# j-moralejo-pinas/dist_classicrl

Measured on AMD Instinct MI355X. Metric: env-steps/sec at 128 agents, 1e6x16 Q-table; 1/2/4/8 GPU + HBM GB/s %peak, higher is better.
Workload: dtype f32

## Files before the change

### dist_classicrl_amd/csrc/qe_rollout_lane.h

```cpp
#pragma once
#include "qe_kernels.h"

namespace qe {

constexpr int LANE_MAX_AGENTS = 512;

template <typename T, int NV>
struct RowV {
    T v[4 * NV];
};

template <int NV>
struct LaneMask {
    using type = uint32_t;
};
template <>
struct LaneMask<16> {
    using type = uint64_t;
};

__device__ __forceinline__ int popc_mask(uint32_t x) { return __popc(x); }
__device__ __forceinline__ int popc_mask(uint64_t x) { return __popcll(x); }

template <int NV>
__device__ __forceinline__ void load_row_lane(RowV<float, NV>& r, const float* q, int64_t row) {
    const float4* p = reinterpret_cast<const float4*>(q + row * (4 * NV));
#pragma unroll
    for (int k = 0; k < NV; ++k) {
        const float4 f = p[k];
        r.v[4 * k] = f.x; r.v[4 * k + 1] = f.y; r.v[4 * k + 2] = f.z; r.v[4 * k + 3] = f.w;
    }
}
template <int NV>
__device__ __forceinline__ void load_row_lane(RowV<double, NV>& r, const double* q, int64_t row) {
    const double2* p = reinterpret_cast<const double2*>(q + row * (4 * NV));
#pragma unroll
    for (int k = 0; k < NV; ++k) {
        const double2 a = p[2 * k], b = p[2 * k + 1];
        r.v[4 * k] = a.x; r.v[4 * k + 1] = a.y; r.v[4 * k + 2] = b.x; r.v[4 * k + 3] = b.y;
    }
}

__device__ __forceinline__ float lane_fmax(float a, float b) { return __builtin_fmaxf(a, b); }
__device__ __forceinline__ double lane_fmax(double a, double b) { return __builtin_fmax(a, b); }

template <bool MASKED, typename T, int NV, typename M>
__device__ __forceinline__ RowV<T, NV> masked_row(const RowV<T, NV>& row, M valid) {
    if constexpr (!MASKED) {
        return row;
    } else {
        RowV<T, NV> r;
#pragma unroll
        for (int j = 0; j < 4 * NV; ++j) r.v[j] = ((valid >> j) & 1) ? row.v[j] : neg_inf<T>();
        return r;
    }
}

template <typename T, int NV>
__device__ __forceinline__ T row_max_lane(const RowV<T, NV>& rowm) {
    T m = neg_inf<T>();
#pragma unroll
    for (int j = 0; j < 4 * NV; ++j) m = lane_fmax(m, rowm.v[j]);
    return m;
}

template <int NV>
__device__ __forceinline__ bool row_nan_lane(const RowV<float, NV>& rowm) {
    typedef float f2 __attribute__((ext_vector_type(2)));
    f2 acc0 = {0.0f, 0.0f}, acc1 = {0.0f, 0.0f};
#pragma unroll
    for (int j = 0; j < 4 * NV; j += 4) {
        const f2 x = {rowm.v[j], rowm.v[j + 1]}, y = {rowm.v[j + 2], rowm.v[j + 3]};
        acc0 = __builtin_elementwise_fma(x, x, acc0);
        acc1 = __builtin_elementwise_fma(y, y, acc1);
    }
    const f2 acc = acc0 + acc1;
    const float s = acc.x + acc.y;
    return s != s;
}
template <int NV>
__device__ __forceinline__ bool row_nan_lane(const RowV<double, NV>& rowm) {
    double acc = 0.0;
#pragma unroll
    for (int j = 0; j < 4 * NV; ++j) acc += rowm.v[j] * rowm.v[j];
    return acc != acc;
}
template <typename T, int NV>
__device__ __forceinline__ T row_max_np_lane(const RowV<T, NV>& rowm) {
    const T m = row_max_lane(rowm);
    return row_nan_lane<NV>(rowm) ? quiet_nan<T>() : m;
}

template <typename T, int NV, int LO, int CNT>
__device__ __forceinline__ T row_pick_tree(const RowV<T, NV>& row, int idx) {
    constexpr int W = 4 * NV;
    if constexpr (CNT == 1) {
        T x = row.v[LO < W ? LO : W - 1];
        asm volatile("" : "+v"(x));
        return x;
    } else {
        const T lo = row_pick_tree<T, NV, LO, CNT / 2>(row, idx);
        const T hi = row_pick_tree<T, NV, LO + CNT / 2, CNT / 2>(row, idx);
        T r = (idx & (CNT / 2)) ? hi : lo;
        asm volatile("" : "+v"(r));
        return r;
    }
}
template <typename T, int NV>
__device__ __forceinline__ T row_pick_lane(const RowV<T, NV>& row, int idx) {
    constexpr int W = 4 * NV;
    constexpr int P = W <= 4 ? 4 : (W <= 8 ? 8 : (W <= 16 ? 16 : (W <= 32 ? 32 : 64)));
    return row_pick_tree<T, NV, 0, P>(row, idx);
}

template <int NV, typename M>
__device__ __forceinline__ int kth_set_bit(M f, int k) {
    constexpr int W = 4 * NV;
    constexpr int P = W <= 4 ? 4 : (W <= 8 ? 8 : (W <= 16 ? 16 : (W <= 32 ? 32 : 64)));
    constexpr int LOG = P == 4 ? 2 : (P == 8 ? 3 : (P == 16 ? 4 : (P == 32 ? 5 : 6)));
    int pos = 0;
#pragma unroll
    for (int lv = 0; lv < LOG; ++lv) {
        const int width = P >> (lv + 1);
        const M low = f & (((M)1 << width) - 1);
        const int c = popc_mask(low);
        const bool hi = k >= c;
        k -= hi ? c : 0;
        f = hi ? (f >> width) : low;
        pos += hi ? width : 0;
    }
    return pos;
}

template <typename T, int NV, typename M, bool PICK = true>
__device__ __forceinline__ int select_lane(const RowV<T, NV>& rowm, M valid, bool explore, uint32_t x1,
                                           uint32_t x2, T* picked, bool nan_max) {
    T m = row_max_lane(rowm);
    if (nan_max) m = quiet_nan<T>();
    M ties = 0;
#pragma unroll
    for (int j = 0; j < 4 * NV; ++j) ties |= (M)(rowm.v[j] == m ? 1u : 0u) << j;
    const M f = explore ? valid : (ties & valid);
    const int total = popc_mask(f);
    int act = -1;
    if (total > 0) act = kth_set_bit<NV>(f, (int)mulhi32(explore ? x1 : x2, (uint32_t)total));
    if constexpr (PICK) *picked = row_pick_lane(rowm, act < 0 ? 0 : act);
    return act;
}

template <class Env, int NV, bool MASKED>
__device__ __forceinline__ typename LaneMask<NV>::type valid_mask_lane(const EnvCtx& ev, int64_t i, int32_t obs) {
    using M = typename LaneMask<NV>::type;
    if constexpr (!MASKED) {
        return ev.A >= 8 * (int)sizeof(M) ? ~(M)0 : (((M)1 << ev.A) - 1);
    } else {
        M m = 0;
#pragma unroll
        for (int sub = 0; sub < NV; ++sub) m |= (M)Env::valid4(ev, i, obs, sub) << (4 * sub);
        return m;
    }
}

template <int CAP>
struct LaneCfg {
    static constexpr int WT = CAP <= 128 ? 4096 : 2048;
    static constexpr int BT = 2048;
};

template <int CAP, bool HELP>
struct LaneLds {
    SlowLdsT<CAP, PERSIST_CACHE_BYTES> slow;
    int wt[4][LaneCfg<CAP>::WT + 1];
    int bt_key[LaneCfg<CAP>::BT];
    unsigned bt_cnt[LaneCfg<CAP>::BT];
    int bt_min[LaneCfg<CAP>::BT];
    uint32_t draws[2][3][HELP ? CAP : 1];
    unsigned long long ep_key[EP_STAGE];
    float ep_ret[EP_STAGE];
    unsigned char pending[CAP];
    alignas(16) unsigned char cold[448];
    unsigned def_bits[CAP / 32];
    unsigned busy[5];
    unsigned ep_n;
    unsigned n_def;
    unsigned complex_;
    int seq_min[2];
};

struct alignas(16) SchedSlot {
    double lr;
    unsigned long long thr;
};
template <int CAP>
struct LaneLdsSlim : LaneLds<CAP, true> {
    SchedSlot sched[2];
    uint2 acct[2][CAP];
};

__device__ __forceinline__ float opaque_copy(float v) {
    float r;
    asm volatile("v_mov_b32 %0, %1" : "=v"(r) : "v"(v));
    return r;
}
__device__ __forceinline__ double opaque_copy(double v) {
    double r;
    asm volatile("v_mov_b64 %0, %1" : "=v"(r) : "v"(v));
    return r;
}

#ifdef QE_EXPERIMENT
#define QX(bit) ((flags >> (20 + (bit))) & 1)
#else
#define QX(bit) 0
#endif
#ifdef QE_STAMPS
#define QL_STAMP(k) do { const long long _n = wall_clock64(); stamp_sum[k] += _n - stamp_last; stamp_last = _n; } while (0)
#else
#define QL_STAMP(k) do { } while (0)
#endif

template <int PENDING_LOADS>
__device__ __forceinline__ void step_barrier() {
    if constexpr (PENDING_LOADS == 0) asm volatile("s_waitcnt vmcnt(0) lgkmcnt(0)\n\ts_barrier" ::: "memory");
    else asm volatile("s_waitcnt vmcnt(%0) lgkmcnt(0)\n\ts_barrier" ::"n"(PENDING_LOADS) : "memory");
}

template <typename T, class Env, int NV, int CAP, bool MASKED, int LEAN = 0, bool HELP = false, bool FULL = false,
          bool SEQ = false>
__global__ __launch_bounds__(HELP ? 4 * CAP : CAP) void k_rollout_lane(InlineSched ,
                                                                       Ctx<T> c, EnvCtx ev, long long steps, int flags) {
    using M = typename LaneMask<NV>::type;
    constexpr int NLOAD = NV * (int)(sizeof(T) / 4);
    constexpr int WT = LaneCfg<CAP>::WT, BT = LaneCfg<CAP>::BT;
    constexpr bool SLIM = HELP && SEQ && FULL && LEAN != 0;
    __shared__ std::conditional_t<SLIM, LaneLdsSlim<CAP>, LaneLds<CAP, HELP>> lds;
    const unsigned long long clk0 = wall_clock64();
    const unsigned long long cyc0 = __builtin_amdgcn_s_memtime();
    if (c.thr == nullptr) {
        const QE_AS4 unsigned char* ka = (const QE_AS4 unsigned char*)__builtin_amdgcn_kernarg_segment_ptr();
        c.thr = (const QE_AS4 unsigned long long*)ka;
        c.lr = (const QE_AS4 double*)(ka + sizeof(unsigned long long) * INLINE_SCHED_STEPS);
    }
    if constexpr (LEAN != 0) { c.mode = 0; c.trace = nullptr; c.rp.s = nullptr; }
    if constexpr (LEAN == 1) c.dlog = nullptr;
#ifdef QE_STAMPS
    long long stamp_sum[8] = {0, 0, 0, 0, 0, 0, 0, 0};
    long long stamp_last = wall_clock64();
    if (threadIdx.x == 0) for (int k = 8; k < 24; ++k) c.vinc[k] = 0.0;
#endif
    const int tid = threadIdx.x;
    const int n_main = HELP ? (int)((c.N + 63) & ~63ll) : (int)blockDim.x;
    const int wave_tid = __builtin_amdgcn_readfirstlane(tid);
    const bool helper = HELP && wave_tid >= n_main && wave_tid < 2 * n_main;
    const bool worker = HELP && wave_tid >= 2 * n_main;
    const int i = helper ? tid - n_main : (worker ? 0 : tid);
    const bool active = FULL ? !(helper || worker) : (!(helper || worker) && i < c.N);
    const int ii = i < c.N ? i : 0;
    Pending<T> p;
    p.n = c.n[ii];
    p.aux = c.aux[ii];
    p.s = 0; p.a = 0; p.pred = 0; p.r = 0.0f; p.term = false;
    float acc = c.acc[ii];
    unsigned long long deferred_total = 0, ep_base = 0;
    unsigned complex_steps = 0;
    int w_next = WT, w_cur = WT, w_prev = WT;
    const int flush_every = 32;
    int flush_in = flush_every;
    for (int k = tid; k < 4 * (WT + 1); k += (int)blockDim.x) (&lds.wt[0][0])[k] = -1;
    for (int k = tid; k < BT; k += (int)blockDim.x) { lds.bt_key[k] = -1; lds.bt_cnt[k] = 0u; lds.bt_min[k] = 0x7FFFFFFF; }
    for (int k = tid; k < CAP; k += (int)blockDim.x) lds.pending[k] = 0;
    if (tid < CAP / 32) lds.def_bits[tid] = 0u;
    static_assert(sizeof(Ctx<T>) <= sizeof(lds.cold), "context stash too small");
    if (tid == 0) {
        *reinterpret_cast<Ctx<T>*>(lds.cold) = c;
        lds.ep_n = 0u; lds.n_def = 0u; lds.complex_ = 0u;
        lds.seq_min[0] = 0x7FFFFFFF; lds.seq_min[1] = 0x7FFFFFFF;
        for (int k = 0; k < 5; ++k) lds.busy[k] = 0u;
        c.ctrl->error = 0u;
        c.ctrl->inv_count = 0u;
    }
    __syncthreads();
    if ((QX(6) && worker) || (QX(7) && helper)) return;

    const bool nan_sel = c.nan_select != 0;
    auto advance = [&](const RowV<T, NV>& row, M valid, long long t1, const U4& x, unsigned long long thr_t1, bool row_nan) {
        const bool explore = (unsigned long long)x.x < thr_t1;
        T picked = p.pred;
        int act = select_lane<T, NV, M, !SLIM>(masked_row<MASKED>(row, valid), valid, explore, x.y, x.z, &picked, nan_sel && row_nan);
        if (act < 0) {
            c.ctrl->error = ERR_EMPTY_CHOICE;
            act = 0;
        }
        const int32_t n = p.n;
        const Transition tr = Env::step(ev, i, n, p.aux, act, c.step0 + (unsigned long long)t1);
        if (c.trace) c.trace[t1 * c.N + i] = act;
        replay_put(c, t1, i, n, act, tr.reward, tr.next_obs, tr.terminated);
        p.s = n; p.a = act; p.pred = picked; p.r = tr.reward; p.term = tr.terminated; p.n = tr.next_obs;
    };
    auto philox_of = [&](long long t1) {
        const unsigned long long step1 = c.step0 + (unsigned long long)t1;
        return philox4x32_10(c.agent_offset + (uint32_t)ii, (uint32_t)step1, (uint32_t)(step1 >> 32), STREAM_POLICY,
                             c.seed_lo, c.seed_hi);
    };
    auto draws = [&](long long t1) {
        if constexpr (HELP) {
            const int slot = (int)(t1 & 1);
            return U4{lds.draws[slot][0][ii], lds.draws[slot][1][ii], lds.draws[slot][2][ii], 0u};
        } else {
            return philox_of(t1);
        }
    };
    auto produce = [&](long long t1) {
        const U4 x = philox_of(t1);
        const int slot = (int)(t1 & 1);
        lds.draws[slot][0][ii] = x.x; lds.draws[slot][1][ii] = x.y; lds.draws[slot][2][ii] = x.z;
        if constexpr (SLIM) {
            if (tid == n_main) {
                lds.sched[slot].lr = c.lr[t1 - 1];
                lds.sched[slot].thr = c.thr[t1 < steps ? t1 : (steps > 0 ? steps - 1 : 0)];
            }
        }
    };
    auto helper_account = [&](long long tk) {
        if constexpr (SLIM) {
            const uint2 rt = lds.acct[tk & 1][ii];
            const bool term = rt.y != 0u;
            acc += __uint_as_float(rt.x);
            const bool ends = term && (flags & FLAG_ACCOUNT);
            const unsigned long long enders = __ballot(ends);
            const float ep_value = acc;
            if (term) acc = 0.0f;
            if (enders) {
                const unsigned rank = __builtin_amdgcn_mbcnt_hi((unsigned)(enders >> 32), __builtin_amdgcn_mbcnt_lo((unsigned)enders, 0u));
                unsigned ep_raw = 0;
                if (ends && rank == 0) ep_raw = atomicAdd(&lds.ep_n, (unsigned)__popcll(enders));
                const unsigned base = __builtin_amdgcn_readlane(ep_raw, __ffsll((long long)enders) - 1);
                if (ends) {
                    const unsigned ep_slot = base + rank;
                    const unsigned long long key = ((unsigned long long)tk << 32) | (unsigned long long)ii;
                    if (ep_slot < (unsigned)EP_STAGE) {
                        lds.ep_key[ep_slot] = key;
                        lds.ep_ret[ep_slot] = ep_value;
                    } else {
                        const Ctx<T>& cc = *reinterpret_cast<const Ctx<T>*>(lds.cold);
                        if ((long long)(ep_base + ep_slot) < cc.ep_cap) {
                            cc.ep_key[ep_base + ep_slot] = key;
                            cc.ep_ret[ep_base + ep_slot] = ep_value;
                        }
                    }
                }
            }
        }
    };
    auto bookkeeping = [&](long long k, bool check_stale) {
        int* const tab_w = lds.wt[(k + 1) & 3];
        const int* const tab_r = lds.wt[k & 3];
        const int* const tab_st = lds.wt[(k + 3) & 3];
        const int32_t rowid = p.n;
        const int h = (int)(mix32((uint32_t)rowid) & (WT - 1));
        const bool need_r = rowid != p.s;
        int o_w = atomicCAS(&tab_w[h], -1, rowid);
        int k_r = need_r ? tab_r[h] : -1;
        int k_st = check_stale ? tab_st[h] : -1;
        int h_w = h, h_r = h, h_st = h;
        bool odd_w = o_w != -1 && o_w != rowid, odd_r = k_r != -1 && k_r != rowid, odd_st = k_st != -1 && k_st != rowid;
        while (__any(odd_w || odd_r || odd_st)) {
            h_w = odd_w ? (h_w + 1) & (WT - 1) : h_w;
            h_r = (h_r + 1) & (WT - 1);
            h_st = (h_st + 1) & (WT - 1);
            const int o2 = atomicCAS(&tab_w[odd_w ? h_w : WT], odd_w ? -1 : -2, rowid);
            const int r2 = tab_r[odd_r ? h_r : WT];
            const int s2 = tab_st[odd_st ? h_st : WT];
            o_w = odd_w ? o2 : o_w; k_r = odd_r ? r2 : k_r; k_st = odd_st ? s2 : k_st;
            odd_w = o_w != -1 && o_w != rowid; odd_r = k_r != -1 && k_r != rowid; odd_st = k_st != -1 && k_st != rowid;
        }
        lds.busy[o_w == rowid ? (int)((k + 1) & 3) : 4] = 1u;
        lds.busy[k_r == rowid ? (int)(k & 3) : 4] = 1u;
        w_prev = w_cur; w_cur = w_next; w_next = h_w;
        return k_st == rowid;
    };

    RowV<T, NV> row;
    bool stale = false;
    T* pred_cell = c.q;
    T pred_pend = 0;
    {
        load_row_lane<NV>(row, c.q, p.n);
        if (active) {
            const M valid0 = valid_mask_lane<Env, NV, MASKED>(ev, i, p.n);
            advance(row, valid0, 0, philox_of(0), c.thr[0], row_nan_lane<NV>(masked_row<MASKED>(row, valid0)));
            int h = (int)(mix32((uint32_t)p.s) & (WT - 1));
            int old = atomicCAS(&lds.wt[0][h], -1, p.s);
            while (old != -1 && old != p.s) {
                h = (h + 1) & (WT - 1);
                old = atomicCAS(&lds.wt[0][h], -1, p.s);
            }
            if (old == p.s) lds.busy[0] = 1u;
            w_next = h;
        }
        if (helper) produce(1);
        __syncthreads();
        if (active) (void)bookkeeping(0, false);
        load_row_lane<NV>(row, c.q, p.n);
        if constexpr (SLIM) {
            pred_cell = c.q + ((int64_t)p.s * (4 * NV) + p.a);
            pred_pend = *pred_cell;
        }
        if constexpr (SLIM) if (active) lds.acct[0][i] = make_uint2(__float_as_uint(p.r), p.term ? 1u : 0u);
    }
    __syncthreads();
    DeltaEntry* dl = c.dlog ? c.dlog + c.dlog_base + ii : nullptr;
    const long long dl_steps = c.dlog ? (c.dlog_cap - c.dlog_base) / c.N : 0;
    int vzero = 0;
    if constexpr (!SLIM) asm volatile("v_mov_b32 %0, 0" : "=v"(vzero));
    double lr_pend = 0.0;
    unsigned long long thr_pend = 0;
    if constexpr (!SLIM) {
        lr_pend = ((const double*)(uintptr_t)c.lr)[vzero];
        thr_pend = ((const unsigned long long*)(uintptr_t)c.thr)[(steps > 1 ? 1 : 0) + vzero];
    }
    for (long long t = 0; t < steps; ++t) {
        const bool last = t + 1 == steps;
        const bool dl_ok = t < dl_steps;
        QL_STAMP(7);
        const bool busy = lds.busy[t & 3] != 0u;
        const U4 x = draws(t + 1);
        double lr_ring = 0.0;
        unsigned long long thr_ring = 0;
        if constexpr (SLIM) { lr_ring = lds.sched[(t + 1) & 1].lr; thr_ring = lds.sched[(t + 1) & 1].thr; }
        if (helper && !last && !QX(5)) produce(t + 2);
        if constexpr (SLIM) if (helper) helper_account(t);
        if (stale && !QX(8)) load_row_lane<NV>(row, c.q, p.n);
        const M valid = valid_mask_lane<Env, NV, MASKED>(ev, ii, p.n);
        QL_STAMP(0);
        int cls = 3;
        int pred_s = -1, pred_n = -1;
        int b_s = -1, b_n = -1;
        if (busy) {
            if (active) {
                auto bt_insert = [&](int32_t rowid) {
                    int h = (int)(mix32((uint32_t)rowid) & (BT - 1));
                    for (;;) {
                        const int old = atomicCAS(&lds.bt_key[h], -1, rowid);
                        if (old == -1 || old == rowid) return h;
                        h = (h + 1) & (BT - 1);
                    }
                };
                b_s = bt_insert(p.s);
                atomicAdd(&lds.bt_cnt[b_s], 1u << 16);
                atomicMin(&lds.bt_min[b_s], i);
                if (p.n != p.s) {
                    b_n = bt_insert(p.n);
                    atomicAdd(&lds.bt_cnt[b_n], 1u);
                    atomicMin(&lds.bt_min[b_n], i);
                }
            }
            barrier_lds();
            if (active) {
                const unsigned cs = lds.bt_cnt[b_s];
                const int ms = lds.bt_min[b_s];
                unsigned cn = 0u;
                int mn = 0x7FFFFFFF;
                const bool has_n = b_n >= 0;
                if (has_n) { cn = lds.bt_cnt[b_n]; mn = lds.bt_min[b_n]; }
                const unsigned w_s = cs >> 16, tot_s = w_s + (cs & 0xFFFFu);
                const unsigned w_n = cn >> 16, tot_n = w_n + (cn & 0xFFFFu);
                bool now = true, sel = true, cx = false;
                if (c.mode == 1) {
                    const bool shared = w_s >= 2u || (w_s == 1u && tot_s >= 2u) || (has_n && w_n >= 1u && tot_n >= 2u);
                    if (shared) { now = false; cx = true; }
                    sel = !(has_n ? w_n > 0u : w_s > 1u);
                } else {
                    if (tot_s > 1u && ms < i) { now = false; pred_s = ms; cx |= tot_s > 2u; }
                    if (has_n) {
                        if (w_n > 0u) {
                            sel = false;
                            if (!p.term && mn < i) { now = false; pred_n = mn; cx |= tot_n > 2u; }
                        }
                    } else if (w_s > 1u) {
                        sel = false;
                    }
                }
                cls = (now ? 1 : 0) | (sel ? 2 : 0);
                if (!now) {
                    lds.pending[i] = 1;
                    atomicAdd(&lds.n_def, 1u);
                    if (cx) lds.complex_ = 1u;
                }
            }
        }
        QL_STAMP(2);
        __builtin_amdgcn_s_waitcnt(0x0F70);
        double lr_t;
        unsigned long long thr_t1;
        if constexpr (SLIM) {
            lr_t = lr_ring;
            thr_t1 = thr_ring;
        } else {
            asm volatile("v_mov_b64 %0, %1" : "=v"(lr_t) : "v"(lr_pend));
            asm volatile("v_mov_b64 %0, %1" : "=v"(thr_t1) : "v"(thr_pend));
            lr_pend = ((const double*)(uintptr_t)c.lr)[(last ? t : t + 1) + vzero];
            thr_pend = ((const unsigned long long*)(uintptr_t)c.thr)[(t + 2 < steps ? t + 2 : steps - 1) + vzero];
        }
        if constexpr (SLIM) p.pred = opaque_copy(pred_pend);
        const float r_t = p.r;
        const bool term_t = p.term;
        bool row_nan = row_nan_lane<NV>(masked_row<MASKED>(row, valid));
        if (active && (cls & 1)) {
            T m = row_max_lane(masked_row<MASKED>(row, valid));
            if (row_nan) m = quiet_nan<T>();
            const int64_t cell = (int64_t)p.s * (4 * NV) + p.a;
            T u;
            const T q1 = Td<T>::apply(p.pred, p.r, m, p.term, make_hyper(c, lr_t), c.mode, &u);
            if (p.n == p.s) row_nan |= q1 != q1;
            if constexpr (SLIM) *pred_cell = q1;
            else if (!QX(1)) c.q[cell] = q1;
            if (dl_ok) *dl = DeltaEntry{(uint32_t)cell, (float)u};
            if (p.n == p.s) {
#pragma unroll
                for (int j = 0; j < 4 * NV; ++j) row.v[j] = j == p.a ? q1 : row.v[j];
            }
        }
        unsigned ep_raw = 0;
        unsigned long long enders = 0;
        float ep_value = 0.0f;
        if (!SLIM && active) {
            acc += r_t;
            enders = __ballot(term_t && (flags & FLAG_ACCOUNT));
            const unsigned rank = __builtin_amdgcn_mbcnt_hi((unsigned)(enders >> 32), __builtin_amdgcn_mbcnt_lo((unsigned)enders, 0u));
            if (term_t) {
                if (rank == 0) ep_raw = atomicAdd(&lds.ep_n, (unsigned)__popcll(enders));
                ep_value = acc;
                acc = 0.0f;
            }
        }
        QL_STAMP(4);
        if (active && !busy && !last) advance(row, valid, t + 1, x, thr_t1, row_nan);
        QL_STAMP(5);

        if (busy) {
#ifdef QE_STAMPS
            const long long ext_t0 = wall_clock64();
#endif
            __syncthreads();
            const int n_def = (int)lds.n_def;
            if (active) {
                lds.bt_key[b_s] = -1; lds.bt_cnt[b_s] = 0u; lds.bt_min[b_s] = 0x7FFFFFFF;
                if (b_n >= 0) { lds.bt_key[b_n] = -1; lds.bt_cnt[b_n] = 0u; lds.bt_min[b_n] = 0x7FFFFFFF; }
            }
#ifdef QE_STAMPS
            if (tid == 0) { c.vinc[16] += 1.0; if (n_def > 0) c.vinc[17] += 1.0; }
#endif
            if (n_def > 0) {
                deferred_total += (unsigned long long)n_def;
                if (lds.complex_) ++complex_steps;
                if constexpr (SEQ) if (lds.complex_) {
                    bool mine = active && !(cls & 1);
                    for (int round = 0; round <= n_def; ++round) {
                        if (mine) atomicMin(&lds.seq_min[round & 1], i);
                        barrier_lds();
                        const int turn = lds.seq_min[round & 1];
                        if (tid == 0) lds.seq_min[(round + 1) & 1] = 0x7FFFFFFF;
                        if (turn == 0x7FFFFFFF) break;
                        if (mine && i == turn) {
                            T m = 0;
                            if (!p.term) {
                                RowV<T, NV> fresh;
                                load_row_lane<NV>(fresh, c.q, p.n);
                                m = row_max_np_lane<T, NV>(masked_row<MASKED>(fresh, valid));
                            }
                            const int64_t cell = (int64_t)p.s * (4 * NV) + p.a;
                            const T q0 = c.q[cell];
                            T u;
                            c.q[cell] = Td<T>::apply(q0, p.r, m, p.term, make_hyper(c, lr_t), 0, &u);
                            log_delta(c, t, i, cell, u);
                            lds.pending[i] = 0;
                            mine = false;
                        }
                        __syncthreads();
                    }
                    if (tid == 0) { lds.seq_min[0] = 0x7FFFFFFF; lds.seq_min[1] = 0x7FFFFFFF; }
                }
                if (!SEQ && lds.complex_) {
                    const Ctx<T>& cold = *reinterpret_cast<const Ctx<T>*>(lds.cold);
                    Ctx<T> cc = c;
                    cc.s = cold.s; cc.a = cold.a; cc.n = cold.n; cc.r = cold.r; cc.term = cold.term;
                    cc.pred = cold.pred; cc.aux = cold.aux; cc.acc = cold.acc;
                    cc.inv_bitmap = cold.inv_bitmap; cc.inv_list = cold.inv_list; cc.vinc = cold.vinc;
                    cc.ctrl = cold.ctrl; cc.ep_key = cold.ep_key; cc.ep_ret = cold.ep_ret; cc.ep_cap = cold.ep_cap;
                    cc.stamps = nullptr; cc.tok = nullptr; cc.adv_bitmap = nullptr; cc.pend_list = nullptr;
                    const bool mine_def = active && !(cls & 1);
                    if (c.mode == 0) {
                        if (mine_def) atomicOr(&lds.def_bits[i >> 5], 1u << (i & 31));
                        barrier_lds();
                        if (mine_def) {
                            int pos = __popc(lds.def_bits[i >> 5] & ((1u << (i & 31)) - 1u));
                            for (int w = 0; w < (i >> 5); ++w) pos += __popc(lds.def_bits[w]);
                            lds.slow.a_agent[pos] = i; lds.slow.a_s[pos] = p.s; lds.slow.a_a[pos] = p.a;
                            lds.slow.a_n[pos] = p.n; lds.slow.a_r[pos] = p.r; lds.slow.a_term[pos] = p.term ? 1 : 0;
                            lds.pending[i] = 0;
                        }
                        barrier_lds();
                        if (tid < CAP / 32) lds.def_bits[tid] = 0u;
                        slow_body<T, Env, CAP, PERSIST_CACHE_BYTES, NV>(
                            cc, ev, FLAG_NO_STAMPS | FLAG_LEARN | FLAG_PRESTAGED, t, n_def, lds.slow);
                    } else {
                        if (mine_def) {
                            cc.s[i] = p.s; cc.a[i] = p.a; cc.pred[i] = p.pred; cc.r[i] = p.r;
                            cc.term[i] = p.term ? 1 : 0; cc.n[i] = p.n; cc.aux[i] = p.aux;
                            atomicOr(&cc.inv_bitmap[i >> 5], 1u << (i & 31));
                            lds.pending[i] = 0;
                        }
                        __syncthreads();
                        (void)build_involved_list(cc, lds.slow.scan);
                        slow_body<T, Env, CAP, PERSIST_CACHE_BYTES, NV>(cc, ev, FLAG_NO_STAMPS | FLAG_LEARN, t, n_def, lds.slow);
                    }
                    __syncthreads();
                } else if (!lds.complex_) {
                    bool mine = active && !(cls & 1);
                    int rounds = 0;
                    while (lds.n_def > 0u && rounds++ <= n_def) {
#ifdef QE_STAMPS
                        if (tid == 0) c.vinc[18] += 1.0;
#endif
                        const bool go = mine && (pred_s < 0 || lds.pending[pred_s] == 0) &&
                                        (pred_n < 0 || lds.pending[pred_n] == 0);
                        barrier_lds();
                        if (go) {
                            T m = 0;
                            if (!p.term) {
                                RowV<T, NV> fresh;
                                load_row_lane<NV>(fresh, c.q, p.n);
                                m = row_max_np_lane<T, NV>(masked_row<MASKED>(fresh, valid));
                            }
                            const int64_t cell = (int64_t)p.s * (4 * NV) + p.a;
                            const T q0 = c.q[cell];
                            T u;
                            c.q[cell] = Td<T>::apply(q0, p.r, m, p.term, make_hyper(c, lr_t), 0, &u);
                            log_delta(c, t, i, cell, u);
                            lds.pending[i] = 0;
                            atomicSub(&lds.n_def, 1u);
                            mine = false;
                        }
                        __syncthreads();
                    }
                    if (tid == 0 && lds.n_def > 0u) reinterpret_cast<const Ctx<T>*>(lds.cold)->ctrl->error = 2u;
                }
            }
            if (active && !last) {
                if (cls != 3 && !((cls & 2) && p.n != p.s)) load_row_lane<NV>(row, c.q, p.n);
                advance(row, valid, t + 1, x, thr_t1, row_nan_lane<NV>(masked_row<MASKED>(row, valid)));
            }
            if (tid == 0) { lds.n_def = 0u; lds.complex_ = 0u; }
            __builtin_amdgcn_s_waitcnt(0x0F70);
#ifdef QE_STAMPS
            if (tid == 0) c.vinc[19] += (double)(wall_clock64() - ext_t0);
#endif
        }
        if (enders) {
            const unsigned base = __builtin_amdgcn_readlane(ep_raw, __ffsll((long long)enders) - 1);
            if ((enders >> (threadIdx.x & 63)) & 1) {
                const unsigned ep_slot = base + __builtin_amdgcn_mbcnt_hi((unsigned)(enders >> 32),
                                                                          __builtin_amdgcn_mbcnt_lo((unsigned)enders, 0u));
                const unsigned long long key = ((unsigned long long)t << 32) | (unsigned long long)i;
                if (ep_slot < (unsigned)EP_STAGE) {
                    lds.ep_key[ep_slot] = key;
                    lds.ep_ret[ep_slot] = ep_value;
                } else {
                    asm volatile("" ::: "memory");
                    const Ctx<T>& cc = *reinterpret_cast<const Ctx<T>*>(lds.cold);
                    if ((long long)(ep_base + ep_slot) < cc.ep_cap) {
                        cc.ep_key[ep_base + ep_slot] = key;
                        cc.ep_ret[ep_base + ep_slot] = ep_value;
                    }
                }
            }
        }
        if (--flush_in == 0 || last) {
            flush_in = flush_every;
            __syncthreads();
            const unsigned staged = lds.ep_n;
            const Ctx<T>& cc = *reinterpret_cast<const Ctx<T>*>(lds.cold);
            unsigned long long* const out_key = cc.ep_key;
            float* const out_ret = cc.ep_ret;
            const long long out_cap = cc.ep_cap;
            for (unsigned k = tid; k < min(staged, (unsigned)EP_STAGE); k += blockDim.x) {
                const unsigned long long pos = ep_base + k;
                if ((long long)pos < out_cap) { out_key[pos] = lds.ep_key[k]; out_ret[pos] = lds.ep_ret[k]; }
            }
            ep_base += staged;
            __syncthreads();
            if (tid == 0) lds.ep_n = 0u;
        }
        QL_STAMP(6);
        if (last) break;
        lds.wt[(t + 3) & 3][w_prev] = -1;
        if (tid == 0) lds.busy[(t + 3) & 3] = 0u;
        asm volatile("" ::: "memory");
        if (!helper && !worker && !QX(0)) load_row_lane<NV>(row, c.q, p.n);
        if constexpr (SLIM) {
            if (!helper && !worker) {
                pred_cell = c.q + ((int64_t)p.s * (4 * NV) + p.a);
                pred_pend = *pred_cell;
            }
        }
        if constexpr (SLIM) if (active) lds.acct[(t + 1) & 1][i] = make_uint2(__float_as_uint(p.r), p.term ? 1u : 0u);
        asm volatile("" ::: "memory");
        if (active && !QX(2)) stale = bookkeeping(t + 1, true);
        QL_STAMP(1);
        if (!QX(4)) step_barrier<NLOAD + (SLIM ? 1 : 0)>();
        if (c.dlog) dl += c.N;
    }
#ifdef QE_STAMPS
    if (tid == 0 && c.vinc) for (int k = 0; k < 8; ++k) c.vinc[k] = (double)stamp_sum[k];
#endif
    const Ctx<T>& cc = *reinterpret_cast<const Ctx<T>*>(lds.cold);
    if (active) {
        cc.n[i] = p.n; cc.aux[i] = p.aux;
        if constexpr (!SLIM) cc.acc[i] = acc;
        if (cc.hb) {
            cc.hb_obs[i] = p.n; cc.hb_aux[i] = p.aux;
            if constexpr (!SLIM) cc.hb_acc[i] = acc;
        }
    }
    if constexpr (SLIM) if (helper) {
        cc.acc[ii] = acc;
        if (cc.hb) cc.hb_acc[ii] = acc;
    }
    if (tid == 0) {
        cc.ctrl->involved_total = deferred_total;
        cc.ctrl->pending_total = complex_steps;
        cc.ctrl->ep_count = ep_base;
        cc.ctrl->t_local = steps;
    }
    if (cc.hb) {
        asm volatile("s_waitcnt vmcnt(0)" ::: "memory");
        __syncthreads();
        if (tid == 0) {
            HostBlock* hb = cc.hb;
            hb->ep_count = ep_base;
            hb->involved_total = deferred_total;
            hb->error = cc.ctrl->error;
            hb->complex_steps = complex_steps;
            hb->clk0 = clk0;
            hb->clk1 = wall_clock64();
            hb->cyc0 = cyc0;
            hb->cyc1 = __builtin_amdgcn_s_memtime();
            __threadfence_system();
            asm volatile("s_waitcnt vmcnt(0)" ::: "memory");
            __hip_atomic_store(&hb->seq, cc.hb_seq, __ATOMIC_RELEASE, __HIP_MEMORY_SCOPE_SYSTEM);
        }
    }
}

}
```

Measured before the change: 31.28 million.

## Resolve non-complex deferred agents in SEQ mode with dependency-driven rounds

```diff
diff --git a/dist_classicrl_amd/csrc/qe_rollout_lane.h b/dist_classicrl_amd/csrc/qe_rollout_lane.h
--- a/dist_classicrl_amd/csrc/qe_rollout_lane.h
+++ b/dist_classicrl_amd/csrc/qe_rollout_lane.h
@@ -452,9 +452,10 @@
                 if (p.n != p.s) {
                     b_n = bt_insert(p.n);
                     atomicAdd(&lds.bt_cnt[b_n], 1u);
-                    atomicMin(&lds.bt_min[b_n], i);
+                    if constexpr (!SEQ) atomicMin(&lds.bt_min[b_n], i);
                 }
             }
+            if constexpr (SEQ) __builtin_amdgcn_s_waitcnt(0x0F70);
             barrier_lds();
             if (active) {
                 const unsigned cs = lds.bt_cnt[b_s];
@@ -470,6 +471,16 @@
                     const bool shared = w_s >= 2u || (w_s == 1u && tot_s >= 2u) || (has_n && w_n >= 1u && tot_n >= 2u);
                     if (shared) { now = false; cx = true; }
                     sel = !(has_n ? w_n > 0u : w_s > 1u);
+                } else if constexpr (SEQ) {
+                    if (w_s > 1u && ms < i) { now = false; pred_s = ms; cx |= tot_s > 2u; }
+                    if (has_n) {
+                        if (w_n > 0u) {
+                            sel = false;
+                            if (!p.term && mn < i) { now = false; pred_n = mn; cx |= tot_n > 2u; }
+                        }
+                    } else if (w_s > 1u) {
+                        sel = false;
+                    }
                 } else {
                     if (tot_s > 1u && ms < i) { now = false; pred_s = ms; cx |= tot_s > 2u; }
                     if (has_n) {
@@ -554,20 +565,35 @@
             if (n_def > 0) {
                 deferred_total += (unsigned long long)n_def;
                 if (lds.complex_) ++complex_steps;
-                if constexpr (SEQ) if (lds.complex_) {
+                if constexpr (SEQ) {
+                    const bool cplx = lds.complex_ != 0u;
+                    const bool single = n_def == 1 && !cplx;
+                    const bool reread_n = pred_n >= 0 || p.n == p.s;
                     bool mine = active && !(cls & 1);
                     for (int round = 0; round <= n_def; ++round) {
-                        if (mine) atomicMin(&lds.seq_min[round & 1], i);
-                        barrier_lds();
-                        const int turn = lds.seq_min[round & 1];
-                        if (tid == 0) lds.seq_min[(round + 1) & 1] = 0x7FFFFFFF;
-                        if (turn == 0x7FFFFFFF) break;
-                        if (mine && i == turn) {
+                        bool go = mine;
+                        if (cplx) {
+                            if (mine) atomicMin(&lds.seq_min[round & 1], i);
+                            barrier_lds();
+                            const int turn = lds.seq_min[round & 1];
+                            if (tid == 0) lds.seq_min[(round + 1) & 1] = 0x7FFFFFFF;
+                            if (turn == 0x7FFFFFFF) break;
+                            go = mine && i == turn;
+                        } else if (!single) {
+                            if (lds.n_def == 0u) break;
+                            go = mine && (pred_s < 0 || lds.pending[pred_s] == 0) && (pred_n < 0 || lds.pending[pred_n] == 0);
+                            barrier_lds();
+                        }
+                        if (go) {
                             T m = 0;
                             if (!p.term) {
-                                RowV<T, NV> fresh;
-                                load_row_lane<NV>(fresh, c.q, p.n);
-                                m = row_max_np_lane<T, NV>(masked_row<MASKED>(fresh, valid));
+                                if (reread_n) {
+                                    RowV<T, NV> fresh;
+                                    load_row_lane<NV>(fresh, c.q, p.n);
+                                    m = row_max_np_lane<T, NV>(masked_row<MASKED>(fresh, valid));
+                                } else {
+                                    m = row_max_np_lane<T, NV>(masked_row<MASKED>(row, valid));
+                                }
                             }
                             const int64_t cell = (int64_t)p.s * (4 * NV) + p.a;
                             const T q0 = c.q[cell];
@@ -575,13 +601,17 @@
                             c.q[cell] = Td<T>::apply(q0, p.r, m, p.term, make_hyper(c, lr_t), 0, &u);
                             log_delta(c, t, i, cell, u);
                             lds.pending[i] = 0;
+                            if (!cplx && !single) atomicSub(&lds.n_def, 1u);
                             mine = false;
                         }
                         __syncthreads();
-                    }
-                    if (tid == 0) { lds.seq_min[0] = 0x7FFFFFFF; lds.seq_min[1] = 0x7FFFFFFF; }
-                }
-                if (!SEQ && lds.complex_) {
+                        if (single) break;
+                    }
+                    if (tid == 0) {
+                        if (cplx) { lds.seq_min[0] = 0x7FFFFFFF; lds.seq_min[1] = 0x7FFFFFFF; }
+                        else if (!single && lds.n_def > 0u) reinterpret_cast<const Ctx<T>*>(lds.cold)->ctrl->error = 2u;
+                    }
+                } else if (!SEQ && lds.complex_) {
                     const Ctx<T>& cold = *reinterpret_cast<const Ctx<T>*>(lds.cold);
                     Ctx<T> cc = c;
                     cc.s = cold.s; cc.a = cold.a; cc.n = cold.n; cc.r = cold.r; cc.term = cold.term;
```

New measurement: 28.74 million. -8.1%, worse.
